# leejaehot/GaussianGrasper

Hardware: AMD Instinct MI355X
Metric: rendered views/sec (fwd+bwd) at 1M Gaussians, 1600x1200, 32-ch feature (higher is better)
Workload: dtype f32; 1 GPU; BASELINE config 4 per-GPU share: 1000000 Gaussians, 1600x1200, SH deg 4 rgb + 32-ch feature + depth + normal images per view (nerfstudio plugin route: the timed callable is FusedGaussianSplattingModel.get_outputs(camera) of gaussiangrasper_amd.plugin (the class train.sh loads, on stub.py's stand-ins for nerfstudio's base model and Cameras) — one fused rasterize operator per view), fwd+bwd, 8 views; route=plugin, deterministic_backward=False, python_gc=gc.freeze() after the warm-up (bench.freeze_gc), view_pipeline=backward of view k beside forward of view k + 1 on two streams, num_gaussians=1000000, feature_dim=32, n_visible=992125, parallelism=view-parallel x1, replicated Gaussians, grad_allreduce_bytes=472000000, grad_allreduce=per parameter, overlapped with the last view's backward

## Files before the change

### gaussiangrasper_amd/csrc/binning.hip

```cpp
#include "scan.h"

__device__ __forceinline__ int64_t dev_count(int64_t n, const int64_t *__restrict__ n_dev) {
    if (n_dev) {
        const int64_t d = *n_dev;
        if (d < n) n = d;
    }
    return n;
}

#define RS_THREADS 256
#define RS_WAVES (RS_THREADS / GG_WAVE)
#ifndef GG_RS_BIG
#define GG_RS_BIG 16
#endif
static inline int rs_items(int64_t n) { return n >= (int64_t)4096 * 1024 ? GG_RS_BIG : 4; }

__global__ __launch_bounds__(256) void count_kernel(int N, const int32_t *__restrict__ nth,
                                                    unsigned long long *__restrict__ out) {
    __shared__ unsigned long long part[4];
    unsigned long long acc = 0;
    for (int i = blockIdx.x * blockDim.x + threadIdx.x; i < N; i += gridDim.x * blockDim.x)
        acc += (unsigned long long)(uint32_t)nth[i];
    for (int off = 32; off > 0; off >>= 1) acc += __shfl_down(acc, off, 64);
    if ((threadIdx.x & 63) == 0) part[threadIdx.x >> 6] = acc;
    __syncthreads();
    if (threadIdx.x == 0) atomicAdd(out, part[0] + part[1] + part[2] + part[3]);
}

extern "C" size_t gg_count_workspace(int num_points) {
    (void)num_points;
    return 0;
}
extern "C" int gg_count_intersects(int N, const int32_t *num_tiles_hit, int64_t *out, void *ws,
                                   size_t ws_bytes, gg_stream_t stream) {
    (void)ws;
    (void)ws_bytes;
    GG_REQUIRE(N >= 0, "num_points < 0");
    GG_REQUIRE(out != nullptr, "null output");
    hipStream_t s = (hipStream_t)stream;
    if (gg_fill_async(out, 0, sizeof(int64_t), s) != hipSuccess) {
        gg_set_error("gg_count_intersects: memset failed");
        return GG_ERR_LAUNCH;
    }
    if (N == 0) return GG_OK;
    GG_REQUIRE(num_tiles_hit != nullptr, "null pointer");
    int blocks = min((N + 255) / 256, 128);
    gg_prof_begin(GG_K_COUNT, s);
    hipLaunchKernelGGL(count_kernel, dim3(blocks), dim3(256), 0, s, N, num_tiles_hit,
                       (unsigned long long *)out);
    gg_prof_end(GG_K_COUNT, s);
    GG_CHECK_LAUNCH();
    return GG_OK;
}

struct DepthSrc {
    const float *depths;
    const int32_t *radii;
};
__device__ __forceinline__ uint32_t depth_key(const DepthSrc d, int64_t idx) {
    return (d.radii[idx] > 0) ? __builtin_bit_cast(uint32_t, d.depths[idx]) : 0xFFFFFFFFu;
}

template <int RS_ITEMS>
__global__ __launch_bounds__(RS_THREADS) void radix_hist_kernel(
    int64_t n, const int64_t *__restrict__ n_dev, const uint32_t *__restrict__ keys, int shift,
    uint32_t mask, int nblocks, uint32_t *__restrict__ G, DepthSrc dsrc) {
    constexpr int RS_TILE = RS_THREADS * RS_ITEMS;
    __shared__ uint32_t hist[256];
    n = dev_count(n, n_dev);
    hist[threadIdx.x] = 0;
    __syncthreads();
    int64_t base = (int64_t)blockIdx.x * RS_TILE;
#pragma unroll 4
    for (int it = 0; it < RS_ITEMS; ++it) {
        int64_t idx = base + (int64_t)it * RS_THREADS + threadIdx.x;
        if (idx < n) atomicAdd(&hist[((dsrc.depths ? depth_key(dsrc, idx) : keys[idx]) >> shift) & mask], 1u);
    }
    __syncthreads();
    G[(size_t)threadIdx.x * nblocks + blockIdx.x] = hist[threadIdx.x];
}

__global__ __launch_bounds__(256) void radix_colscan_kernel(int nblocks, uint32_t *__restrict__ G,
                                                            uint32_t *__restrict__ totals) {
    __shared__ uint32_t wsum[4];
    __shared__ uint32_t carry_s;
    uint32_t *row = G + (size_t)blockIdx.x * nblocks;
    const int lane = threadIdx.x & 63, wave = threadIdx.x >> 6;
    if (threadIdx.x == 0) carry_s = 0;
    __syncthreads();
    for (int start = 0; start < nblocks; start += 256) {
        int i = start + threadIdx.x;
        uint32_t v = (i < nblocks) ? row[i] : 0u;
        uint32_t incl = v;
        for (int off = 1; off < 64; off <<= 1) {
            uint32_t t = __shfl_up(incl, off, 64);
            if (lane >= off) incl += t;
        }
        if (lane == 63) wsum[wave] = incl;
        __syncthreads();
        uint32_t wpre = 0;
        for (int w = 0; w < wave; ++w) wpre += wsum[w];
        uint32_t carry = carry_s;
        if (i < nblocks) row[i] = carry + wpre + incl - v;
        __syncthreads();
        if (threadIdx.x == 255) carry_s = carry + wpre + incl;
        __syncthreads();
    }
    if (threadIdx.x == 0) totals[blockIdx.x] = carry_s;
}

template <int RS_ITEMS>
__global__ __launch_bounds__(RS_THREADS) void radix_scatter_kernel(
    int64_t n, const int64_t *__restrict__ n_dev, const uint32_t *__restrict__ keys_in,
    const uint32_t *__restrict__ vals_in, uint32_t *__restrict__ keys_out,
    uint32_t *__restrict__ vals_out, int shift, uint32_t mask, int nblocks,
    const uint32_t *__restrict__ G, const uint32_t *__restrict__ totals, DepthSrc dsrc) {
    constexpr int RS_TILE = RS_THREADS * RS_ITEMS;
    n = dev_count(n, n_dev);
    const int nbits = 32 - __builtin_clz(mask | 1u);
    __shared__ uint32_t whist[RS_WAVES][256];
    __shared__ uint32_t digit_base[256];
    __shared__ uint32_t wsum[4];
    const int tid = threadIdx.x, lane = tid & 63, wave = tid >> 6;
    {
        uint32_t v = totals[tid];
        uint32_t incl = v;
        for (int off = 1; off < 64; off <<= 1) {
            uint32_t t = __shfl_up(incl, off, 64);
            if (lane >= off) incl += t;
        }
        if (lane == 63) wsum[wave] = incl;
        for (int w = 0; w < RS_WAVES; ++w) whist[w][tid] = 0;
        __syncthreads();
        uint32_t wpre = 0;
        for (int w = 0; w < wave; ++w) wpre += wsum[w];
        digit_base[tid] = wpre + incl - v + G[(size_t)tid * nblocks + blockIdx.x];
    }
    __syncthreads();

    const int64_t wbase = (int64_t)blockIdx.x * RS_TILE + (int64_t)wave * (GG_WAVE * RS_ITEMS);
    uint32_t key[RS_ITEMS], val[RS_ITEMS], rank[RS_ITEMS];
    const uint64_t lt_mask = (lane == 0) ? 0ull : (~0ull >> (64 - lane));
#pragma unroll
    for (int it = 0; it < RS_ITEMS; ++it) {
        int64_t idx = wbase + (int64_t)it * GG_WAVE + lane;
        bool valid = idx < n;
        key[it] = valid ? (dsrc.depths ? depth_key(dsrc, idx) : keys_in[idx]) : 0u;
        val[it] = valid ? (dsrc.depths ? (uint32_t)idx : vals_in[idx]) : 0u;
    }
#pragma unroll
    for (int it = 0; it < RS_ITEMS; ++it) {
        int64_t idx = wbase + (int64_t)it * GG_WAVE + lane;
        bool valid = idx < n;
        uint32_t d = (key[it] >> shift) & mask;
        uint64_t peers = __ballot(valid);
#pragma unroll
        for (int b = 0; b < 8; ++b) {
            if (b < nbits) {
                bool bit = (d >> b) & 1u;
                uint64_t m = __ballot(bit);
                peers &= bit ? m : ~m;
            }
        }
        uint32_t cnt = (uint32_t)__popcll(peers);
        uint32_t before = (uint32_t)__popcll(peers & lt_mask);
        uint32_t old = 0u;
        if (valid && before == 0) old = atomicAdd(&whist[wave][d], cnt);
        old = __shfl(old, (int)__builtin_ctzll(peers | (1ull << 63)), 64);
        rank[it] = old + before;
    }
    __syncthreads();
// ... 2 lines not shown
    {
        uint32_t run = 0;
        for (int w = 0; w < RS_WAVES; ++w) {
            uint32_t c = whist[w][tid];
            whist[w][tid] = run;
            run += c;
        }
        uint32_t incl = run;
        for (int off = 1; off < 64; off <<= 1) {
            uint32_t u = __shfl_up(incl, off, 64);
            if (lane >= off) incl += u;
        }
        if (lane == 63) wsum[wave] = incl;
        __syncthreads();
        uint32_t wpre = 0;
        for (int w = 0; w < wave; ++w) wpre += wsum[w];
        lstart[tid] = wpre + incl - run;
    }
    __syncthreads();
#pragma unroll
    for (int it = 0; it < RS_ITEMS; ++it) {
        int64_t idx = wbase + (int64_t)it * GG_WAVE + lane;
        if (idx < n) {
            uint32_t d = (key[it] >> shift) & mask;
            uint32_t lp = lstart[d] + whist[wave][d] + rank[it];
            skey[lp] = key[it];
            sval[lp] = val[it];
        }
    }
    __syncthreads();
    const int64_t left = n - (int64_t)blockIdx.x * RS_TILE;
    const int count = (int)(left < RS_TILE ? left : RS_TILE);
    for (int jj = tid; jj < count; jj += RS_THREADS) {
        const uint32_t k = skey[jj];
        const uint32_t d = (k >> shift) & mask;
        const uint32_t dst = digit_base[d] + ((uint32_t)jj - lstart[d]);
        keys_out[dst] = k;
        vals_out[dst] = sval[jj];
    }
}


typedef unsigned long long u64;
#define DB_BLOCKS 64
#define DB_THREADS 1024
#define DB_CAP 512
#define DB_MAX_BUCKETS 32768
static inline int db_buckets(int N) {
    int nb = 256;
    while (nb < DB_MAX_BUCKETS && nb * 64 < N) nb <<= 1;
    return nb;
}
struct DbRange {
    uint32_t kmin;
    u64 mul;
};
struct DbParts {
    const uint32_t *lo, *hi;
    int n;
};
__device__ __forceinline__ DbRange db_range_of(const DbParts mm, int nb, uint32_t *s_mm ) {
    const int tid = threadIdx.x;
    if (tid < 64) {
        uint32_t lo = 0xFFFFFFFFu, hi = 0u;
        for (int i = tid; i < mm.n; i += 64) {
            lo = min(lo, mm.lo[i]);
            hi = max(hi, mm.hi[i]);
        }
        for (int off = 32; off > 0; off >>= 1) {
            lo = min(lo, (uint32_t)__shfl_xor((int)lo, off, 64));
            hi = max(hi, (uint32_t)__shfl_xor((int)hi, off, 64));
        }
        if (tid == 0) { s_mm[0] = lo; s_mm[1] = hi; }
    }
    __syncthreads();
    DbRange r;
    const uint32_t lo = s_mm[0], hi = s_mm[1];
    r.kmin = lo;
    const u64 span = hi >= lo ? (u64)(hi - lo) + 1ull : 1ull;
    r.mul = (((u64)nb) << 32) / span;
    return r;
}
__device__ __forceinline__ uint32_t db_bucket(const DbRange r, uint32_t key, int nb) {
    if (key == 0xFFFFFFFFu) return (uint32_t)nb;
    return min((uint32_t)(((u64)(key - r.kmin) * r.mul) >> 32), (uint32_t)(nb - 1));
}
__global__ __launch_bounds__(256) void db_range_kernel(int N, DepthSrc dsrc, uint32_t *__restrict__ mm) {
    __shared__ uint32_t s_lo[4], s_hi[4];
    uint32_t lo = 0xFFFFFFFFu, hi = 0u;
    const int stride = 256 * gridDim.x;
    for (int i = blockIdx.x * 256 + threadIdx.x; i < N; i += 4 * stride) {
        uint32_t k[4];
#pragma unroll
        for (int u = 0; u < 4; ++u) k[u] = (i + u * stride < N) ? depth_key(dsrc, i + u * stride) : 0xFFFFFFFFu;
#pragma unroll
        for (int u = 0; u < 4; ++u)
            if (k[u] != 0xFFFFFFFFu) { lo = min(lo, k[u]); hi = max(hi, k[u]); }
    }
    for (int off = 32; off > 0; off >>= 1) {
        lo = min(lo, (uint32_t)__shfl_xor((int)lo, off, 64));
        hi = max(hi, (uint32_t)__shfl_xor((int)hi, off, 64));
    }
    if ((threadIdx.x & 63) == 0) { s_lo[threadIdx.x >> 6] = lo; s_hi[threadIdx.x >> 6] = hi; }
    __syncthreads();
    if (threadIdx.x == 0) {
        mm[blockIdx.x] = min(min(s_lo[0], s_lo[1]), min(s_lo[2], s_lo[3]));
        mm[gridDim.x + blockIdx.x] = max(max(s_hi[0], s_hi[1]), max(s_hi[2], s_hi[3]));
    }
}
#define DB_BOX_MAX 1023
struct DbGeom {
    const float *xys;
    int tiles_x, tiles_y;
};
__device__ __forceinline__ void db_box(const DbGeom g, const DepthSrc d, int i, uint32_t &cnt, uint32_t &box) {
    const int rad = d.radii[i];
    cnt = 0u;
    box = 1u << 20;
    if (rad > 0) {
        int x0, y0, x1, y1;
        gg_tile_bbox(g.xys[2 * (size_t)i], g.xys[2 * (size_t)i + 1], (float)rad, g.tiles_x, g.tiles_y, x0, y0, x1, y1);
        const int bw = x1 - x0;
        if (bw > 0 && y1 > y0) {
            cnt = (uint32_t)(bw * (y1 - y0));
            box = (uint32_t)x0 | ((uint32_t)y0 << 10) | ((uint32_t)bw << 20);
        }
    }
}
template <bool SCATTER>
__global__ __launch_bounds__(DB_THREADS) void db_walk_kernel(int N, int nb, DepthSrc dsrc, DbGeom geom,
                                                             const DbParts mm, uint32_t *__restrict__ G,
                                                             const uint32_t *__restrict__ start, uint4 *__restrict__ recs,
                                                             int32_t *__restrict__ zero = nullptr, int nzero = 0) {
    for (int i = blockIdx.x * DB_THREADS + threadIdx.x; i < nzero; i += DB_BLOCKS * DB_THREADS) zero[i] = 0;
    extern __shared__ uint32_t s_hist[];
    uint32_t *s_mm = s_hist + nb + 1;
    const DbRange r = db_range_of(mm, nb, s_mm);
    const int per = (N + DB_BLOCKS - 1) / DB_BLOCKS;
    const int lo = blockIdx.x * per, hi = min(N, lo + per);
    uint32_t *row = G + (size_t)blockIdx.x * (nb + 1);
    for (int b = threadIdx.x; b <= nb; b += DB_THREADS) s_hist[b] = SCATTER ? start[b] + row[b] : 0u;
    __syncthreads();
    for (int i = lo + threadIdx.x; i < hi; i += 4 * DB_THREADS) {
        uint32_t k[4], cnt[4], box[4];
#pragma unroll
        for (int u = 0; u < 4; ++u) {
            const int iu = i + u * DB_THREADS;
            k[u] = iu < hi ? depth_key(dsrc, iu) : 0u;
            cnt[u] = box[u] = 0u;
            if (SCATTER && iu < hi) db_box(geom, dsrc, iu, cnt[u], box[u]);
        }
#pragma unroll
        for (int u = 0; u < 4; ++u) {
            if (i + u * DB_THREADS < hi) {
                const uint32_t pos = atomicAdd(&s_hist[db_bucket(r, k[u], nb)], 1u);
                if (SCATTER && k[u] != 0xFFFFFFFFu)
                    recs[pos] = make_uint4(k[u], (uint32_t)(i + u * DB_THREADS), cnt[u], box[u]);
            }
        }
    }
    if (!SCATTER) {
        __syncthreads();
        for (int b = threadIdx.x; b <= nb; b += DB_THREADS) row[b] = s_hist[b];
    }
}
__global__ __launch_bounds__(256) void db_prefix_kernel(int nb, uint32_t *__restrict__ G, uint32_t *__restrict__ total) {
    const int b = blockIdx.x * 256 + threadIdx.x;
    if (b > nb) return;
    uint32_t run = 0;
    uint32_t c[DB_BLOCKS];
#pragma unroll
    for (int k = 0; k < DB_BLOCKS; ++k) c[k] = G[(size_t)k * (nb + 1) + b];
#pragma unroll
    for (int k = 0; k < DB_BLOCKS; ++k) {
        G[(size_t)k * (nb + 1) + b] = run;
        run += c[k];
    }
    total[b] = run;
}
__global__ __launch_bounds__(1024) void db_scan_kernel(int n, uint32_t *__restrict__ v) {
    __shared__ uint32_t s_w[2][16];
    const int tid = threadIdx.x, lane = tid & 63, wave = tid >> 6;
    uint32_t carry = 0u;
    int round = 0;
    for (int base = 0; base < n; base += 4 * 4096) {
        uint32_t x[4][4];
#pragma unroll
        for (int q = 0; q < 4; ++q)
#pragma unroll
            for (int k = 0; k < 4; ++k) {
                const int i = base + 4096 * q + 4 * tid + k;
                x[q][k] = i < n ? v[i] : 0u;
            }
#pragma unroll
        for (int q = 0; q < 4; ++q, ++round) {
            if (base + 4096 * q >= n) break;
            const uint32_t mine = x[q][0] + x[q][1] + x[q][2] + x[q][3];
            uint32_t incl = mine;
#pragma unroll
            for (int off = 1; off < 64; off <<= 1) {
                const uint32_t t = __shfl_up(incl, off, 64);
                if (lane >= off) incl += t;
            }
            uint32_t *sw = s_w[round & 1];
            if (lane == 63) sw[wave] = incl;
            __syncthreads();
            uint32_t ex = carry + incl - mine, all = 0u;
#pragma unroll
            for (int w = 0; w < 16; ++w) {
                const uint32_t t = sw[w];
                if (w < wave) ex += t;
                all += t;
            }
            carry += all;
#pragma unroll
            for (int k = 0; k < 4; ++k) {
                const int i = base + 4096 * q + 4 * tid + k;
                if (i < n) v[i] = ex;
                ex += x[q][k];
            }
        }
    }
    if (tid == 0) v[n] = carry;
}

__device__ __forceinline__ void db_ce(u64 &a, u64 &b) {
    const bool sw = b < a;
    const u64 lo = sw ? b : a, hi = sw ? a : b;
    a = lo;
    b = hi;
}
__device__ __forceinline__ void db_bitonic64(u64 *buf, const int n) {
    constexpr int NB = 8, LNB = 3, THREADS = 64;
    const int tid = threadIdx.x & 63;
    int P = NB;
    while (P < n) P <<= 1;
    const u64 INF = ~0ull;
    for (int blk = tid; blk * NB < n; blk += THREADS) {
        u64 v[NB];
#pragma unroll
        for (int r = 0; r < NB; ++r) v[r] = (NB * blk + r < n) ? buf[NB * blk + r] : INF;
#pragma unroll
        for (int k = 2; k <= NB; k <<= 1) {
#pragma unroll
            for (int i = 0; i < NB / 2; ++i) {
                const int b2 = i / (k / 2), off = i % (k / 2);
                db_ce(v[b2 * k + off], v[b2 * k + k - 1 - off]);
            }
#pragma unroll
            for (int j = k >> 2; j >= 1; j >>= 1)
#pragma unroll
                for (int i = 0; i < NB / 2; ++i) {
                    const int lo = ((i & ~(j - 1)) << 1) | (i & (j - 1));
                    db_ce(v[lo], v[lo + j]);
                }
        }
#pragma unroll
        for (int r = 0; r < NB; ++r)
            if (NB * blk + r < n) buf[NB * blk + r] = v[r];
    }
    { __builtin_amdgcn_fence(__ATOMIC_ACQ_REL, "workgroup"); __builtin_amdgcn_wave_barrier(); }
    for (int k = 2 * NB, lk = LNB + 1; k <= P; k <<= 1, ++lk) {
        const int hk = k >> 1;
        for (int i = tid; i < (P >> 1); i += THREADS) {
            const int blk = i >> (lk - 1), off = i & (hk - 1);
            const int lo = blk * k + off, hi = blk * k + k - 1 - off;
            if (hi < n) {
                const u64 a = buf[lo], b = buf[hi];
                if (b < a) { buf[lo] = b; buf[hi] = a; }
            }
        }
        { __builtin_amdgcn_fence(__ATOMIC_ACQ_REL, "workgroup"); __builtin_amdgcn_wave_barrier(); }
        for (int j = k >> 2; j >= NB; j >>= 1) {
            for (int i = tid; i < (P >> 1); i += THREADS) {
                const int lo = ((i & ~(j - 1)) << 1) | (i & (j - 1)), hi = lo + j;
                if (hi < n) {
// ... 177 lines not shown
#pragma unroll
                for (int r = 0; r < DB_ITEMS; ++r) key[r] = (64 * r < nv) ? buf[64 * r + lane] : ~0ull;
            }
            db_wsync();
        };
#pragma nounroll
        for (int round = 0; round < 2; ++round) {
#pragma nounroll
            for (int pb = round == 0 ? 4 : 0; pb < 8; ++pb) pass(8 * pb);
            if (round == 1) break;
            {
                DB_LIM(nv);
#pragma unroll
                for (int r = 0; r < DB_ITEMS; ++r)
                    if (64 * r < nv) buf[64 * r + lane] = key[r];
            }
            db_wsync();
            bool bad = false;
            {
                DB_LIM(nv);
#pragma unroll
                for (int r = 0; r < DB_ITEMS; ++r)
                    if (64 * r + 1 < nv) {
                        const u64 nx = buf[64 * r + lane + 1];
                        bad = bad || ((uint32_t)(nx >> 32) == (uint32_t)(key[r] >> 32) && (uint32_t)nx < (uint32_t)key[r]);
                    }
            }
            db_wsync();
            if (__ballot(bad) == 0ull) break;
        }
#undef DB_LIM
#pragma unroll
        for (int r = 0; r < DB_ITEMS; ++r) gid[r] = (uint32_t)key[r];
    } else {
        for (int i = lane; i < n; i += 64) {
            const uint4 rc = recs[s0 + i];
            pairs[s0 + i] = ((u64)rc.x << 32) | rc.y;
        }
        db_wsync();
        db_bitonic64(pairs + s0, n);
    }
    uint32_t carry = 0;
    for (int c0 = 0; c0 < n; c0 += DB_CAP) {
        if (n > DB_CAP) {
#pragma unroll
            for (int r = 0; r < DB_ITEMS; ++r) gid[r] = (c0 + 64 * r + lane < n) ? (uint32_t)pairs[s0 + c0 + 64 * r + lane] : 0u;
        }
#pragma unroll
        for (int r = 0; r < DB_ITEMS; ++r) {
            const int p = c0 + 64 * r + lane;
            if (c0 + 64 * r < n) {
                const bool valid = p < n;
                const uint32_t g = min(gid[r], (uint32_t)(N - 1));
                uint32_t c = cntv[r], bx = boxv[r];
                if (!carried) {
                    c = 0u;
                    bx = 1u << 20;
                    if (valid) db_box(geom, dsrc, (int)g, c, bx);
                }
                if (!valid) c = 0u;
                uint32_t incl = c;
#pragma unroll
                for (int off = 1; off < 64; off <<= 1) {
                    const uint32_t u = __shfl_up(incl, off, 64);
                    if (lane >= off) incl += u;
                }
                if (valid) {
                    order[s0 + p] = g;
                    einfo[s0 + p] = make_uint4(carry + incl - c, (uint32_t)b, bx, c);
                }
                carry += __shfl(incl, 63, 64);
            }
        }
    }
    if (lane == 0) bucket_sum[b] = carry;
}

__global__ __launch_bounds__(256) void emit_kernel(int N, const uint32_t *__restrict__ order,
                                                   const uint4 *__restrict__ einfo,
                                                   const uint32_t *__restrict__ bucket_base,
                                                   const uint32_t *__restrict__ visible, int tiles_x,
                                                   int64_t I, const int64_t *__restrict__ I_dev,
                                                   uint32_t *__restrict__ tkeys,
                                                   uint32_t *__restrict__ tvals) {
    __shared__ uint32_t s_rel[4][64];
    I = dev_count(I, I_dev);
    __shared__ int4 s_box[4][64];
    const int lane = threadIdx.x & 63, wave = threadIdx.x >> 6;
    const int r = blockIdx.x * blockDim.x + threadIdx.x;
    uint32_t g = 0, cnt = 0, off = 0;
    int x0 = 0, y0 = 0, bw = 1;
    if (r < N && (uint32_t)r < *visible) {
        g = min(order[r], (uint32_t)(N - 1));
        const uint4 e = einfo[r];
        off = e.x + bucket_base[e.y];
        x0 = (int)(e.z & 1023u);
        y0 = (int)((e.z >> 10) & 1023u);
        bw = max(1, (int)(e.z >> 20));
        cnt = e.w;
    }
    uint32_t incl = cnt;
    for (int d = 1; d < 64; d <<= 1) {
        uint32_t u = __shfl_up(incl, d, 64);
        if (lane >= d) incl += u;
    }
    const uint32_t total = __shfl(incl, 63, 64);
    const uint32_t base = __shfl(off, 0, 64);
    s_rel[wave][lane] = incl - cnt;
    s_box[wave][lane] = make_int4(x0, y0, bw, (int)g);
    __builtin_amdgcn_wave_barrier();
    const uint32_t *rel = s_rel[wave];
    for (uint32_t j = lane; j < total; j += 64) {
        int lo = 0;
#pragma unroll
        for (int step = 32; step > 0; step >>= 1)
            if (rel[lo + step] <= j) lo += step;
        const int4 b = s_box[wave][lo];
        const uint32_t k = j - rel[lo];
        const uint32_t row = k / (uint32_t)b.z;
        const int64_t cur = (int64_t)base + j;
        if (cur < I) {
            tkeys[cur] = (uint32_t)((b.y + (int)row) * tiles_x + b.x + (int)(k - row * (uint32_t)b.z));
            tvals[cur] = (uint32_t)b.w;
        }
    }
}

__global__ __launch_bounds__(256) void tile_bins_kernel(int64_t I, const int64_t *__restrict__ I_dev,
                                                        const uint32_t *__restrict__ tkeys_sorted,
                                                        uint32_t num_tiles,
                                                        int32_t *__restrict__ tile_bins,
                                                        int32_t *__restrict__ tile_out) {
    I = dev_count(I, I_dev);
    int64_t i = (int64_t)blockIdx.x * blockDim.x + threadIdx.x;
    if (i >= I) return;
    uint32_t cur = tkeys_sorted[i];
    if (tile_out) tile_out[i] = (int32_t)cur;
    const bool cur_ok = cur < num_tiles;
    if (i == 0 && cur_ok) tile_bins[2 * cur] = 0;
    if (i == I - 1 && cur_ok) tile_bins[2 * cur + 1] = (int32_t)I;
    if (i > 0) {
        uint32_t prev = tkeys_sorted[i - 1];
        if (prev != cur) {
            if (prev < num_tiles) tile_bins[2 * prev + 1] = (int32_t)i;
            if (cur_ok) tile_bins[2 * cur] = (int32_t)i;
        }
    }
}

static int radix_nblocks(int64_t n) {
    const int64_t tile = (int64_t)RS_THREADS * rs_items(n);
    return (int)((n + tile - 1) / tile);
}

struct BinWs {
    uint32_t *order;
    uint4 *einfo;
    uint32_t *G;
    uint32_t *totals;
    uint32_t *tkeyA, *tkeyB, *tvalTmp;
    uint4 *recs;
    u64 *pairs;
    uint32_t *dbG;
    uint32_t *dbStart;
    uint32_t *dbBase;
    uint32_t *dbmm;
    size_t bytes;
};
static BinWs bin_ws_layout(void *ws, int N, int64_t I) {
    BinWs w;
    size_t off = 0;
    auto take = [&](size_t nbytes) {
        char *p = ws ? (char *)ws + off : nullptr;
        off += gg_align_up(nbytes, 256);
        return (uint32_t *)p;
    };
    size_t n = (size_t)(N > 0 ? N : 1), i = (size_t)(I > 0 ? I : 1);
    w.order = take(4 * n);
    w.einfo = (uint4 *)take(16 * n);
    int nb = max(radix_nblocks(N), radix_nblocks(I));
    w.G = take(4 * 256 * (size_t)(nb + 1));
    w.totals = take(4 * 256);
    w.tkeyA = take(4 * i);
    w.tkeyB = take(4 * i);
    w.tvalTmp = take(4 * i);
    const size_t nbk = (size_t)db_buckets(N);
    w.recs = (uint4 *)take(16 * n);
    w.pairs = (u64 *)take(8 * n);
    w.dbG = take(4 * DB_BLOCKS * (nbk + 1));
    w.dbStart = take(4 * (nbk + 2));
    w.dbBase = take(4 * (nbk + 1));
    w.dbmm = take(4 * 2 * 256);
    w.bytes = off;
    return w;
}
extern "C" size_t gg_bin_sort_workspace(int num_points, int64_t num_intersects) {
    return bin_ws_layout(nullptr, num_points, num_intersects).bytes;
}

static void radix_pass(int64_t n, const int64_t *n_dev, const uint32_t *kin, const uint32_t *vin,
                       uint32_t *kout, uint32_t *vout, int shift, uint32_t mask, BinWs &w, hipStream_t s,
                       DepthSrc dsrc = DepthSrc{nullptr, nullptr}) {
    int nb = radix_nblocks(n);
    if (rs_items(n) != 4)
        hipLaunchKernelGGL(radix_hist_kernel<GG_RS_BIG>, dim3(nb), dim3(RS_THREADS), 0, s, n, n_dev, kin, shift,
                           mask, nb, w.G, dsrc);
    else
        hipLaunchKernelGGL(radix_hist_kernel<4>, dim3(nb), dim3(RS_THREADS), 0, s, n, n_dev, kin, shift,
                           mask, nb, w.G, dsrc);
    hipLaunchKernelGGL(radix_colscan_kernel, dim3(256), dim3(256), 0, s, nb, w.G, w.totals);
    if (rs_items(n) != 4)
        hipLaunchKernelGGL(radix_scatter_kernel<GG_RS_BIG>, dim3(nb), dim3(RS_THREADS), 0, s, n, n_dev, kin, vin,
                           kout, vout, shift, mask, nb, w.G, w.totals, dsrc);
    else
        hipLaunchKernelGGL(radix_scatter_kernel<4>, dim3(nb), dim3(RS_THREADS), 0, s, n, n_dev, kin, vin,
                           kout, vout, shift, mask, nb, w.G, w.totals, dsrc);
}

static int bin_sort_impl(int N, int64_t I, const int64_t *I_dev, const float *xys, const float *depths,
                         const int32_t *radii, const int32_t *num_tiles_hit, int tiles_x, int tiles_y,
                         int32_t *gaussian_ids_sorted, int32_t *tile_bins, int32_t *isect_tile_sorted,
                         void *ws, size_t ws_bytes, gg_stream_t stream, const uint32_t *range_lo = nullptr,
                         const uint32_t *range_hi = nullptr, int range_parts = 0) {
    GG_REQUIRE(N >= 0 && I >= 0, "negative size");
    GG_REQUIRE(tiles_x > 0 && tiles_y > 0, "empty tile grid");
    GG_REQUIRE(tiles_x <= DB_BOX_MAX && tiles_y <= DB_BOX_MAX, "tile grid beyond 1023 x 1023 (images beyond 16 368 pixels a side)");
    GG_REQUIRE(I < (int64_t)1 << 31, "num_intersects must fit int32 (tile_bins are int32)");
    GG_REQUIRE(tile_bins != nullptr, "null tile_bins");
    hipStream_t s = (hipStream_t)stream;
    const int T = tiles_x * tiles_y;
    if (N == 0 || I == 0) {
        if (gg_fill_async(tile_bins, 0, sizeof(int32_t) * 2 * (size_t)T, s) != hipSuccess) {
            gg_set_error("gg_bin_sort: memset failed");
            return GG_ERR_LAUNCH;
        }
        return GG_OK;
    }
    GG_REQUIRE(xys && depths && radii && num_tiles_hit && gaussian_ids_sorted, "null pointer");
    BinWs w = bin_ws_layout(ws, N, I);
    if (ws == nullptr || ws_bytes < w.bytes) {
        gg_set_error("gg_bin_sort: workspace too small (%zu < %zu)", ws_bytes, w.bytes);
        return GG_ERR_WORKSPACE;
    }
    gg_prof_begin(GG_K_BIN_SORT, s);
    const int nbk = db_buckets(N);
    const DepthSrc dsrc{depths, radii};
    const size_t walk_lds = sizeof(uint32_t) * ((size_t)nbk + 1 + 2);
    if (walk_lds > 64 * 1024) {
        (void)hipFuncSetAttribute((const void *)db_walk_kernel<false>, hipFuncAttributeMaxDynamicSharedMemorySize, (int)walk_lds);
        (void)hipFuncSetAttribute((const void *)db_walk_kernel<true>, hipFuncAttributeMaxDynamicSharedMemorySize, (int)walk_lds);
    }
    uint32_t *order = w.order;
    DbParts mm{w.dbmm, w.dbmm + 256, 256};
    if (range_lo && range_hi && range_parts > 0)
        mm = DbParts{range_lo, range_hi, range_parts};
    else
        hipLaunchKernelGGL(db_range_kernel, dim3(256), dim3(256), 0, s, N, dsrc, w.dbmm);
    const DbGeom geom{xys, tiles_x, tiles_y};
    hipLaunchKernelGGL(db_walk_kernel<false>, dim3(DB_BLOCKS), dim3(DB_THREADS), walk_lds, s, N, nbk, dsrc, geom, mm,
                       w.dbG, (const uint32_t *)nullptr, (uint4 *)nullptr, tile_bins, 2 * T);
    hipLaunchKernelGGL(db_prefix_kernel, dim3((nbk + 1 + 255) / 256), dim3(256), 0, s, nbk, w.dbG, w.dbStart);
    hipLaunchKernelGGL(db_scan_kernel, dim3(1), dim3(1024), 0, s, nbk, w.dbStart);
    hipLaunchKernelGGL(db_walk_kernel<true>, dim3(DB_BLOCKS), dim3(DB_THREADS), walk_lds, s, N, nbk, dsrc, geom, mm,
                       w.dbG, (const uint32_t *)w.dbStart, w.recs, (int32_t *)nullptr, 0);
    hipLaunchKernelGGL(db_sort_kernel, dim3((nbk + DB_WPB - 1) / DB_WPB), dim3(64 * DB_WPB), 0, s, N, nbk,
                       (const uint32_t *)w.dbStart, (const uint4 *)w.recs, w.pairs, dsrc, geom, order, w.einfo, w.dbBase);
    hipLaunchKernelGGL(db_scan_kernel, dim3(1), dim3(1024), 0, s, nbk, w.dbBase);
    int tile_bits = 1;
    while ((1 << tile_bits) < T) ++tile_bits;
    int passes = (tile_bits + 7) / 8;
    uint32_t *out_vals = (uint32_t *)gaussian_ids_sorted;
    uint32_t *kcur = w.tkeyA, *kalt = w.tkeyB;
    uint32_t *vcur = (passes % 2 == 0) ? out_vals : w.tvalTmp;
    uint32_t *valt = (passes % 2 == 0) ? w.tvalTmp : out_vals;
    if (!I_dev) {
        (void)gg_fill_async(kcur, 0xFF, sizeof(uint32_t) * (size_t)I, s);
        (void)gg_fill_async(vcur, 0, sizeof(uint32_t) * (size_t)I, s);
    }
    hipLaunchKernelGGL(emit_kernel, dim3((N + 255) / 256), dim3(256), 0, s, N, (const uint32_t *)order,
                       (const uint4 *)w.einfo, (const uint32_t *)w.dbBase, (const uint32_t *)(w.dbStart + nbk), tiles_x, I,
                       I_dev, kcur, vcur);
    const int per_pass = (tile_bits + passes - 1) / passes;
    for (int pass = 0; pass < passes; ++pass) {
        int bits = min(per_pass, tile_bits - per_pass * pass);
        radix_pass(I, I_dev, kcur, vcur, kalt, valt, per_pass * pass, (1u << bits) - 1u, w, s);
        uint32_t *t = kcur; kcur = kalt; kalt = t;
        t = vcur; vcur = valt; valt = t;
    }
    hipLaunchKernelGGL(tile_bins_kernel, dim3((unsigned)((I + 255) / 256)), dim3(256), 0, s, I, I_dev, kcur,
                       (uint32_t)T, tile_bins, isect_tile_sorted);
    gg_prof_end(GG_K_BIN_SORT, s);
    GG_CHECK_LAUNCH();
    return GG_OK;
}

extern "C" int gg_bin_sort_status(int N, int64_t I, const void *ws, size_t ws_bytes, gg_stream_t stream) {
    GG_REQUIRE(N >= 0 && I >= 0, "negative size");
    (void)ws;
    (void)ws_bytes;
    if (hipStreamSynchronize((hipStream_t)stream) != hipSuccess) {
        gg_set_error("gg_bin_sort_status: stream synchronisation failed");
        return GG_ERR_LAUNCH;
    }
    return GG_OK;
}

extern "C" int gg_bin_sort(int N, int64_t I, const float *xys, const float *depths,
                           const int32_t *radii, const int32_t *num_tiles_hit, int tiles_x,
                           int tiles_y, int32_t *gaussian_ids_sorted, int32_t *tile_bins,
                           int32_t *isect_tile_sorted, void *ws, size_t ws_bytes,
                           gg_stream_t stream) {
    return bin_sort_impl(N, I, nullptr, xys, depths, radii, num_tiles_hit, tiles_x, tiles_y,
                         gaussian_ids_sorted, tile_bins, isect_tile_sorted, ws, ws_bytes, stream);
}

extern "C" int gg_bin_sort_dev(int N, int64_t capacity, const int64_t *num_intersects_dev,
                               const float *xys, const float *depths, const int32_t *radii,
                               const int32_t *num_tiles_hit, int tiles_x, int tiles_y,
                               int32_t *gaussian_ids_sorted, int32_t *tile_bins,
                               int32_t *isect_tile_sorted, void *ws, size_t ws_bytes,
                               gg_stream_t stream) {
    GG_REQUIRE(num_intersects_dev != nullptr, "null num_intersects_dev");
    GG_REQUIRE(capacity >= 1, "capacity < 1");
    return bin_sort_impl(N, capacity, num_intersects_dev, xys, depths, radii, num_tiles_hit, tiles_x,
                         tiles_y, gaussian_ids_sorted, tile_bins, isect_tile_sorted, ws, ws_bytes, stream);
}

extern "C" int gg_bin_sort_dev_ex(int N, int64_t capacity, const int64_t *num_intersects_dev,
                                  const float *xys, const float *depths, const int32_t *radii,
                                  const int32_t *num_tiles_hit, int tiles_x, int tiles_y,
                                  int32_t *gaussian_ids_sorted, int32_t *tile_bins,
                                  int32_t *isect_tile_sorted, void *ws, size_t ws_bytes,
                                  const uint32_t *depth_bits_min, const uint32_t *depth_bits_max, int range_parts,
                                  gg_stream_t stream) {
    GG_REQUIRE(num_intersects_dev != nullptr, "null num_intersects_dev");
    GG_REQUIRE(capacity >= 1, "capacity < 1");
    GG_REQUIRE(range_parts == 0 || (depth_bits_min && depth_bits_max && range_parts > 0), "range parts without arrays");
    return bin_sort_impl(N, capacity, num_intersects_dev, xys, depths, radii, num_tiles_hit, tiles_x,
                         tiles_y, gaussian_ids_sorted, tile_bins, isect_tile_sorted, ws, ws_bytes, stream,
                         depth_bits_min, depth_bits_max, range_parts);
}

size_t gg_sort_pairs_workspace(int64_t n) {
// ... 32 lines not shown
```

Measured before the change: 638.9 views/s.

## Replace per-tile radix sort with coarse block binning plus fine in-block tile expansion

New measurement: 639.8 views/s (median of 6 runs). Within noise of the previous version (+0.1%).

```diff
diff --git a/gaussiangrasper_amd/csrc/binning.hip b/gaussiangrasper_amd/csrc/binning.hip
--- a/gaussiangrasper_amd/csrc/binning.hip
+++ b/gaussiangrasper_amd/csrc/binning.hip
@@ -68,6 +68,7 @@
     constexpr int RS_TILE = RS_THREADS * RS_ITEMS;
     __shared__ uint32_t hist[256];
     n = dev_count(n, n_dev);
+    if ((int64_t)blockIdx.x * RS_TILE >= n) return;
     hist[threadIdx.x] = 0;
     __syncthreads();
     int64_t base = (int64_t)blockIdx.x * RS_TILE;
@@ -81,16 +82,19 @@
 }
 
 __global__ __launch_bounds__(256) void radix_colscan_kernel(int nblocks, uint32_t *__restrict__ G,
-                                                            uint32_t *__restrict__ totals) {
+                                                            uint32_t *__restrict__ totals, int64_t n,
+                                                            const int64_t *__restrict__ n_dev, int tile) {
     __shared__ uint32_t wsum[4];
     __shared__ uint32_t carry_s;
     uint32_t *row = G + (size_t)blockIdx.x * nblocks;
+    n = dev_count(n, n_dev);
+    const int active = (int)min((int64_t)nblocks, (n + tile - 1) / tile);
     const int lane = threadIdx.x & 63, wave = threadIdx.x >> 6;
     if (threadIdx.x == 0) carry_s = 0;
     __syncthreads();
-    for (int start = 0; start < nblocks; start += 256) {
+    for (int start = 0; start < active; start += 256) {
         int i = start + threadIdx.x;
-        uint32_t v = (i < nblocks) ? row[i] : 0u;
+        uint32_t v = (i < active) ? row[i] : 0u;
         uint32_t incl = v;
         for (int off = 1; off < 64; off <<= 1) {
             uint32_t t = __shfl_up(incl, off, 64);
@@ -101,7 +105,7 @@
         uint32_t wpre = 0;
         for (int w = 0; w < wave; ++w) wpre += wsum[w];
         uint32_t carry = carry_s;
-        if (i < nblocks) row[i] = carry + wpre + incl - v;
+        if (i < active) row[i] = carry + wpre + incl - v;
         __syncthreads();
         if (threadIdx.x == 255) carry_s = carry + wpre + incl;
         __syncthreads();
@@ -117,6 +121,7 @@
     const uint32_t *__restrict__ G, const uint32_t *__restrict__ totals, DepthSrc dsrc) {
     constexpr int RS_TILE = RS_THREADS * RS_ITEMS;
     n = dev_count(n, n_dev);
+    if ((int64_t)blockIdx.x * RS_TILE >= n) return;
     const int nbits = 32 - __builtin_clz(mask | 1u);
     __shared__ uint32_t whist[RS_WAVES][256];
     __shared__ uint32_t digit_base[256];
@@ -225,7 +230,7 @@
     return nb;
 }
 struct DbRange {
-    uint32_t kmin;
+    uint32_t kmin, kmax;
     u64 mul;
 };
 struct DbParts {
@@ -250,13 +255,15 @@
     DbRange r;
     const uint32_t lo = s_mm[0], hi = s_mm[1];
     r.kmin = lo;
+    r.kmax = hi >= lo ? hi : lo;
     const u64 span = hi >= lo ? (u64)(hi - lo) + 1ull : 1ull;
     r.mul = (((u64)nb) << 32) / span;
     return r;
 }
 __device__ __forceinline__ uint32_t db_bucket(const DbRange r, uint32_t key, int nb) {
     if (key == 0xFFFFFFFFu) return (uint32_t)nb;
-    return min((uint32_t)(((u64)(key - r.kmin) * r.mul) >> 32), (uint32_t)(nb - 1));
+    const uint32_t k = min(max(key, r.kmin), r.kmax);
+    return min((uint32_t)(((u64)(k - r.kmin) * r.mul) >> 32), (uint32_t)(nb - 1));
 }
 __global__ __launch_bounds__(256) void db_range_kernel(int N, DepthSrc dsrc, uint32_t *__restrict__ mm) {
     __shared__ uint32_t s_lo[4], s_hi[4];
@@ -285,6 +292,7 @@
 struct DbGeom {
     const float *xys;
     int tiles_x, tiles_y;
+    int lbx, lby;
 };
 __device__ __forceinline__ void db_box(const DbGeom g, const DepthSrc d, int i, uint32_t &cnt, uint32_t &box) {
     const int rad = d.radii[i];
@@ -293,9 +301,10 @@
     if (rad > 0) {
         int x0, y0, x1, y1;
         gg_tile_bbox(g.xys[2 * (size_t)i], g.xys[2 * (size_t)i + 1], (float)rad, g.tiles_x, g.tiles_y, x0, y0, x1, y1);
-        const int bw = x1 - x0;
-        if (bw > 0 && y1 > y0) {
-            cnt = (uint32_t)(bw * (y1 - y0));
+        const int bw = x1 - x0, bh = y1 - y0;
+        if (bw > 0 && bh > 0) {
+            const int nblk = (((x1 - 1) >> g.lbx) - (x0 >> g.lbx) + 1) * (((y1 - 1) >> g.lby) - (y0 >> g.lby) + 1);
+            cnt = (uint32_t)nblk | ((uint32_t)bh << 16);
             box = (uint32_t)x0 | ((uint32_t)y0 << 10) | ((uint32_t)bw << 20);
         }
     }
@@ -351,7 +360,14 @@
     }
     total[b] = run;
 }
-__global__ __launch_bounds__(1024) void db_scan_kernel(int n, uint32_t *__restrict__ v) {
+struct TileOut {
+    int2 *bins;
+    int64_t I;
+    const int64_t *I_dev;
+    int32_t *ids, *tiles;
+};
+__global__ __launch_bounds__(1024) void db_scan_kernel(int n, uint32_t *__restrict__ v, TileOut to = TileOut{}) {
+    const int64_t L = to.bins ? dev_count(to.I, to.I_dev) : 0;
     __shared__ uint32_t s_w[2][16];
     const int tid = threadIdx.x, lane = tid & 63, wave = tid >> 6;
     uint32_t carry = 0u;
@@ -389,12 +405,23 @@
 #pragma unroll
             for (int k = 0; k < 4; ++k) {
                 const int i = base + 4096 * q + 4 * tid + k;
-                if (i < n) v[i] = ex;
+                if (i < n) {
+                    v[i] = ex;
+                    if (to.bins) {
+                        const int64_t e = ex, f = e + x[q][k];
+                        to.bins[i] = x[q][k] ? make_int2((int)min(e, L), (int)min(f, L)) : make_int2(0, 0);
+                    }
+                }
                 ex += x[q][k];
             }
         }
     }
     if (tid == 0) v[n] = carry;
+    if (to.bins)
+        for (int64_t p = (int64_t)carry + tid; p < L; p += 1024) {
+            to.ids[p] = 0;
+            if (to.tiles) to.tiles[p] = -1;
+        }
 }
 
 __device__ __forceinline__ void db_ce(u64 &a, u64 &b) {
@@ -678,13 +705,13 @@
             if (c0 + 64 * r < n) {
                 const bool valid = p < n;
                 const uint32_t g = min(gid[r], (uint32_t)(N - 1));
-                uint32_t c = cntv[r], bx = boxv[r];
+                uint32_t cw = cntv[r], bx = boxv[r];
                 if (!carried) {
-                    c = 0u;
+                    cw = 0u;
                     bx = 1u << 20;
-                    if (valid) db_box(geom, dsrc, (int)g, c, bx);
+                    if (valid) db_box(geom, dsrc, (int)g, cw, bx);
                 }
-                if (!valid) c = 0u;
+                const uint32_t c = valid ? cw & 0xFFFFu : 0u;
                 uint32_t incl = c;
 #pragma unroll
                 for (int off = 1; off < 64; off <<= 1) {
@@ -693,7 +720,7 @@
                 }
                 if (valid) {
                     order[s0 + p] = g;
-                    einfo[s0 + p] = make_uint4(carry + incl - c, (uint32_t)b, bx, c);
+                    einfo[s0 + p] = make_uint4(carry + incl - c, (uint32_t)b, bx, cw >> 16);
                 }
                 carry += __shfl(incl, 63, 64);
             }
@@ -702,28 +729,40 @@
     if (lane == 0) bucket_sum[b] = carry;
 }
 
-__global__ __launch_bounds__(256) void emit_kernel(int N, const uint32_t *__restrict__ order,
-                                                   const uint4 *__restrict__ einfo,
-                                                   const uint32_t *__restrict__ bucket_base,
-                                                   const uint32_t *__restrict__ visible, int tiles_x,
-                                                   int64_t I, const int64_t *__restrict__ I_dev,
-                                                   uint32_t *__restrict__ tkeys,
-                                                   uint32_t *__restrict__ tvals) {
+struct BinBlocks {
+    int lbx, lby;
+    int nbx;
+    int nblocks;
+};
+__device__ __forceinline__ int fs_seg(int bt) { return max(512, 8 * bt); }
+#define FS_BATCH 8
+
+__global__ __launch_bounds__(256) void coarse_emit_kernel(int N, const uint32_t *__restrict__ order,
+                                                          const uint4 *__restrict__ einfo,
+                                                          const uint32_t *__restrict__ bucket_base, int nbk,
+                                                          const uint32_t *__restrict__ visible, BinBlocks bb, int64_t I,
+                                                          const int64_t *__restrict__ I_dev, uint32_t *__restrict__ ckeys,
+                                                          uint32_t *__restrict__ cvals, int64_t *__restrict__ ccount) {
     __shared__ uint32_t s_rel[4][64];
-    I = dev_count(I, I_dev);
     __shared__ int4 s_box[4][64];
+    const int64_t L = dev_count(I, I_dev);
+    if (blockIdx.x == 0 && threadIdx.x == 0) *ccount = min((int64_t)bucket_base[nbk], L);
     const int lane = threadIdx.x & 63, wave = threadIdx.x >> 6;
     const int r = blockIdx.x * blockDim.x + threadIdx.x;
     uint32_t g = 0, cnt = 0, off = 0;
-    int x0 = 0, y0 = 0, bw = 1;
+    int x0 = 0, y0 = 0, x1 = 0, y1 = 0, nbx = 1;
     if (r < N && (uint32_t)r < *visible) {
         g = min(order[r], (uint32_t)(N - 1));
         const uint4 e = einfo[r];
         off = e.x + bucket_base[e.y];
         x0 = (int)(e.z & 1023u);
         y0 = (int)((e.z >> 10) & 1023u);
-        bw = max(1, (int)(e.z >> 20));
-        cnt = e.w;
+        x1 = x0 + (int)(e.z >> 20) - 1;
+        y1 = y0 + (int)e.w - 1;
+        if (e.w > 0u) {
+            nbx = (x1 >> bb.lbx) - (x0 >> bb.lbx) + 1;
+            cnt = (uint32_t)(nbx * ((y1 >> bb.lby) - (y0 >> bb.lby) + 1));
+        }
     }
     uint32_t incl = cnt;
     for (int d = 1; d < 64; d <<= 1) {
@@ -733,9 +772,11 @@
     const uint32_t total = __shfl(incl, 63, 64);
     const uint32_t base = __shfl(off, 0, 64);
     s_rel[wave][lane] = incl - cnt;
-    s_box[wave][lane] = make_int4(x0, y0, bw, (int)g);
+    s_box[wave][lane] = make_int4(x0 | (x1 << 16), y0 | (y1 << 16), nbx, (int)g);
     __builtin_amdgcn_wave_barrier();
     const uint32_t *rel = s_rel[wave];
+    const int BW = 1 << bb.lbx, BH = 1 << bb.lby;
+    const int sx1 = 8 + bb.lbx, sy0 = 8 + 2 * bb.lbx, sy1 = 8 + 2 * bb.lbx + bb.lby;
     for (uint32_t j = lane; j < total; j += 64) {
         int lo = 0;
 #pragma unroll
@@ -743,40 +784,144 @@
             if (rel[lo + step] <= j) lo += step;
         const int4 b = s_box[wave][lo];
         const uint32_t k = j - rel[lo];
-        const uint32_t row = k / (uint32_t)b.z;
+        const int row = (int)(k / (uint32_t)b.z), col = (int)k - row * b.z;
+        const int bx0 = b.x & 0xFFFF, bx1 = b.x >> 16, by0 = b.y & 0xFFFF, by1 = b.y >> 16;
+        const int bx = (bx0 >> bb.lbx) + col, by = (by0 >> bb.lby) + row;
+        const int X = bx << bb.lbx, Y = by << bb.lby;
+        const uint32_t key = (uint32_t)(by * bb.nbx + bx) | ((uint32_t)(max(bx0, X) - X) << 8) |
+                             ((uint32_t)(min(bx1, X + BW - 1) - X) << sx1) | ((uint32_t)(max(by0, Y) - Y) << sy0) |
+                             ((uint32_t)(min(by1, Y + BH - 1) - Y) << sy1);
         const int64_t cur = (int64_t)base + j;
-        if (cur < I) {
-            tkeys[cur] = (uint32_t)((b.y + (int)row) * tiles_x + b.x + (int)(k - row * (uint32_t)b.z));
-            tvals[cur] = (uint32_t)b.w;
-        }
-    }
-}
-
-__global__ __launch_bounds__(256) void tile_bins_kernel(int64_t I, const int64_t *__restrict__ I_dev,
-                                                        const uint32_t *__restrict__ tkeys_sorted,
-                                                        uint32_t num_tiles,
-                                                        int32_t *__restrict__ tile_bins,
-                                                        int32_t *__restrict__ tile_out) {
-    I = dev_count(I, I_dev);
-    int64_t i = (int64_t)blockIdx.x * blockDim.x + threadIdx.x;
-    if (i >= I) return;
-    uint32_t cur = tkeys_sorted[i];
-    if (tile_out) tile_out[i] = (int32_t)cur;
-    const bool cur_ok = cur < num_tiles;
-    if (i == 0 && cur_ok) tile_bins[2 * cur] = 0;
-    if (i == I - 1 && cur_ok) tile_bins[2 * cur + 1] = (int32_t)I;
-    if (i > 0) {
-        uint32_t prev = tkeys_sorted[i - 1];
-        if (prev != cur) {
-            if (prev < num_tiles) tile_bins[2 * prev + 1] = (int32_t)i;
-            if (cur_ok) tile_bins[2 * cur] = (int32_t)i;
-        }
-    }
-}
-
-static int radix_nblocks(int64_t n) {
-    const int64_t tile = (int64_t)RS_THREADS * rs_items(n);
+        if (cur < L) {
+            ckeys[cur] = key;
+            cvals[cur] = (uint32_t)b.w;
+        }
+    }
+}
+
+__device__ __forceinline__ bool fs_locate(const uint32_t *__restrict__ totals, int S, int seg, int &b, uint32_t &lo,
+                                          uint32_t &hi, int &first) {
+    __shared__ uint32_t s_cs[256], s_sf[257], s_w[2][4];
+    const int tid = threadIdx.x, lane = tid & 63, wave = tid >> 6;
+    const uint32_t c = totals[tid], ns = (c + (uint32_t)S - 1u) / (uint32_t)S;
+    uint32_t ic = c, is = ns;
+    for (int off = 1; off < 64; off <<= 1) {
+        const uint32_t u = __shfl_up(ic, off, 64), v = __shfl_up(is, off, 64);
+        if (lane >= off) { ic += u; is += v; }
+    }
+    if (lane == 63) { s_w[0][wave] = ic; s_w[1][wave] = is; }
+    __syncthreads();
+    uint32_t pc = 0, ps = 0;
+    for (int w = 0; w < wave; ++w) { pc += s_w[0][w]; ps += s_w[1][w]; }
+    s_cs[tid] = pc + ic - c;
+    s_sf[tid] = ps + is - ns;
+    if (tid == 255) s_sf[256] = ps + is;
+    __syncthreads();
+    if ((uint32_t)seg >= s_sf[256]) return false;
+    int k = 0;
+#pragma unroll
+    for (int step = 128; step > 0; step >>= 1)
+        if (k + step < 256 && s_sf[k + step] <= (uint32_t)seg) k += step;
+    b = k;
+    first = (int)s_sf[k];
+    lo = s_cs[k] + (uint32_t)(seg - first) * (uint32_t)S;
+    hi = min(lo + (uint32_t)S, s_cs[k] + totals[k]);
+    return true;
+}
+
+template <bool WRITE>
+__global__ __launch_bounds__(256) void fine_kernel(const uint32_t *__restrict__ ckeys, const uint32_t *__restrict__ cvals,
+                                                   const uint32_t *__restrict__ totals, BinBlocks bb, int tiles_x,
+                                                   int tiles_y, uint32_t *__restrict__ cnt, uint32_t *__restrict__ tot,
+                                                   int64_t I, const int64_t *__restrict__ I_dev,
+                                                   int32_t *__restrict__ ids, int32_t *__restrict__ tiles_out) {
+    const int lane = threadIdx.x & 63;
+    const int BW = 1 << bb.lbx, BH = 1 << bb.lby, BT = BW * BH, S = fs_seg(BT);
+    const int seg = blockIdx.x * 4 + (threadIdx.x >> 6);
+    int b, first;
+    uint32_t lo, hi;
+    if (!fs_locate(totals, S, seg, b, lo, hi, first)) return;
+    const int64_t L = WRITE ? dev_count(I, I_dev) : 0;
+    const int X = (b % bb.nbx) << bb.lbx, Y = (b / bb.nbx) << bb.lby;
+    const int sx1 = 8 + bb.lbx, sy0 = 8 + 2 * bb.lbx, sy1 = 8 + 2 * bb.lbx + bb.lby;
+    const uint64_t lt_mask = (lane == 0) ? 0ull : (~0ull >> (64 - lane));
+    for (int c0 = 0; c0 < BT; c0 += 64) {
+        const int lt = c0 + lane;
+        const int tx = X + (lt & (BW - 1)), ty = Y + (lt >> bb.lbx);
+        const bool own = lt < BT && tx < tiles_x && ty < tiles_y;
+        const int tile = own ? ty * tiles_x + tx : 0;
+        uint32_t run = 0;
+        if (WRITE && own) {
+            run = tot[tile];
+#pragma unroll 8
+            for (int s = first; s < seg; ++s) run += cnt[(size_t)s * BT + lt];
+        }
+        const int r0 = c0 >> bb.lbx, r1 = min(c0 + 64, BT) >> bb.lbx;
+        for (uint32_t b0 = lo; b0 < hi; b0 += 64 * FS_BATCH) {
+            uint32_t kk[FS_BATCH], gg[FS_BATCH];
+#pragma unroll
+            for (int q = 0; q < FS_BATCH; ++q) {
+                const uint32_t i = b0 + 64u * q + (uint32_t)lane;
+                kk[q] = i < hi ? ckeys[i] : 0u;
+                gg[q] = (WRITE && i < hi) ? cvals[i] : 0u;
+            }
+#pragma unroll
+            for (int q = 0; q < FS_BATCH; ++q) {
+                if (b0 + 64u * q >= hi) break;
+                const bool v = b0 + 64u * q + (uint32_t)lane < hi;
+                const uint32_t k = kk[q], gid = gg[q];
+                const int lx0 = (int)((k >> 8) & (uint32_t)(BW - 1)), lx1 = (int)((k >> sx1) & (uint32_t)(BW - 1));
+                const int ly0 = (int)((k >> sy0) & (uint32_t)(BH - 1)), ly1 = (int)((k >> sy1) & (uint32_t)(BH - 1));
+#pragma nounroll
+                for (int ry = r0; ry < r1; ++ry) {
+                    const bool rowc = v && ly0 <= ry && ry <= ly1;
+                    if (__ballot(rowc) == 0ull) continue;
+#pragma nounroll
+                    for (int rx = 0; rx < BW; ++rx) {
+                        const bool on = rowc && lx0 <= rx && rx <= lx1;
+                        const uint64_t m = __ballot(on);
+                        const int owner = ((ry << bb.lbx) | rx) - c0;
+                        if (WRITE && m != 0ull) {
+                            const uint32_t p = (uint32_t)__builtin_amdgcn_readlane((int)run, owner) +
+                                               (uint32_t)__popcll(m & lt_mask);
+                            if (on && (int64_t)p < L) {
+                                ids[p] = (int32_t)gid;
+                                if (tiles_out) tiles_out[p] = (Y + ry) * tiles_x + X + rx;
+                            }
+                        }
+                        if (lane == owner) run += (uint32_t)__popcll(m);
+                    }
+                }
+            }
+        }
+        if (!WRITE && lt < BT) {
+            cnt[(size_t)seg * BT + lt] = run;
+            if (run) atomicAdd(&tot[tile], run);
+        }
+    }
+}
+
+static int radix_nblocks(int64_t n, int items) {
+    const int64_t tile = (int64_t)RS_THREADS * items;
     return (int)((n + tile - 1) / tile);
+}
+static int radix_nblocks(int64_t n) { return radix_nblocks(n, rs_items(n)); }
+static int coarse_items(int64_t I) { return rs_items(I / 4); }
+
+static BinBlocks bin_blocks(int tiles_x, int tiles_y) {
+    BinBlocks b{3, 2, 0, 0};
+    for (;;) {
+        b.nbx = (tiles_x + (1 << b.lbx) - 1) >> b.lbx;
+        b.nblocks = b.nbx * ((tiles_y + (1 << b.lby) - 1) >> b.lby);
+        if (b.nblocks <= 256) return b;
+        if (b.lbx <= b.lby) ++b.lbx; else ++b.lby;
+    }
+}
+static int fs_seg_h(int bt) { return max(512, 8 * bt); }
+#define FS_MAX_BT 4096
+static int64_t fs_segments(int64_t L, const BinBlocks &bb) {
+    const int S = fs_seg_h(1 << (bb.lbx + bb.lby));
+    return (L + S - 1) / S + bb.nblocks;
 }
 
 struct BinWs {
@@ -784,7 +929,10 @@
     uint4 *einfo;
     uint32_t *G;
     uint32_t *totals;
-    uint32_t *tkeyA, *tkeyB, *tvalTmp;
+    uint32_t *ckA, *cvA, *ckB, *cvB;
+    int64_t *ccount;
+    uint32_t *fcnt;
+    uint32_t *ttot;
     uint4 *recs;
     u64 *pairs;
     uint32_t *dbG;
@@ -804,12 +952,15 @@
     size_t n = (size_t)(N > 0 ? N : 1), i = (size_t)(I > 0 ? I : 1);
     w.order = take(4 * n);
     w.einfo = (uint4 *)take(16 * n);
-    int nb = max(radix_nblocks(N), radix_nblocks(I));
-    w.G = take(4 * 256 * (size_t)(nb + 1));
+    w.G = take(4 * 256 * (size_t)(max(radix_nblocks(I), radix_nblocks(I, coarse_items(I))) + 1));
     w.totals = take(4 * 256);
-    w.tkeyA = take(4 * i);
-    w.tkeyB = take(4 * i);
-    w.tvalTmp = take(4 * i);
+    w.ckA = take(4 * i);
+    w.cvA = take(4 * i);
+    w.ckB = take(4 * i);
+    w.cvB = take(4 * i);
+    w.ccount = (int64_t *)take(8);
+    w.fcnt = take(4 * (i / 8 + 257 * (size_t)FS_MAX_BT));
+    w.ttot = take(4 * ((size_t)DB_BOX_MAX * DB_BOX_MAX + 1));
     const size_t nbk = (size_t)db_buckets(N);
     w.recs = (uint4 *)take(16 * n);
     w.pairs = (u64 *)take(8 * n);
@@ -826,16 +977,18 @@
 
 static void radix_pass(int64_t n, const int64_t *n_dev, const uint32_t *kin, const uint32_t *vin,
                        uint32_t *kout, uint32_t *vout, int shift, uint32_t mask, BinWs &w, hipStream_t s,
-                       DepthSrc dsrc = DepthSrc{nullptr, nullptr}) {
-    int nb = radix_nblocks(n);
-    if (rs_items(n) != 4)
+                       DepthSrc dsrc = DepthSrc{nullptr, nullptr}, int items = 0) {
+    if (items == 0) items = rs_items(n);
+    const int nb = radix_nblocks(n, items);
+    if (items != 4)
         hipLaunchKernelGGL(radix_hist_kernel<GG_RS_BIG>, dim3(nb), dim3(RS_THREADS), 0, s, n, n_dev, kin, shift,
                            mask, nb, w.G, dsrc);
     else
         hipLaunchKernelGGL(radix_hist_kernel<4>, dim3(nb), dim3(RS_THREADS), 0, s, n, n_dev, kin, shift,
                            mask, nb, w.G, dsrc);
-    hipLaunchKernelGGL(radix_colscan_kernel, dim3(256), dim3(256), 0, s, nb, w.G, w.totals);
-    if (rs_items(n) != 4)
+    hipLaunchKernelGGL(radix_colscan_kernel, dim3(256), dim3(256), 0, s, nb, w.G, w.totals, n, n_dev,
+                       RS_THREADS * items);
+    if (items != 4)
         hipLaunchKernelGGL(radix_scatter_kernel<GG_RS_BIG>, dim3(nb), dim3(RS_THREADS), 0, s, n, n_dev, kin, vin,
                            kout, vout, shift, mask, nb, w.G, w.totals, dsrc);
     else
@@ -868,6 +1021,13 @@
         gg_set_error("gg_bin_sort: workspace too small (%zu < %zu)", ws_bytes, w.bytes);
         return GG_ERR_WORKSPACE;
     }
+    const BinBlocks bb = bin_blocks(tiles_x, tiles_y);
+    const int BT = 1 << (bb.lbx + bb.lby);
+    const int64_t nseg = fs_segments(I, bb);
+    if ((size_t)nseg * BT > I / 8 + 257 * (size_t)FS_MAX_BT) {
+        gg_set_error("gg_bin_sort: segment counts exceed their workspace");
+        return GG_ERR_WORKSPACE;
+    }
     gg_prof_begin(GG_K_BIN_SORT, s);
     const int nbk = db_buckets(N);
     const DepthSrc dsrc{depths, radii};
@@ -882,39 +1042,32 @@
         mm = DbParts{range_lo, range_hi, range_parts};
     else
         hipLaunchKernelGGL(db_range_kernel, dim3(256), dim3(256), 0, s, N, dsrc, w.dbmm);
-    const DbGeom geom{xys, tiles_x, tiles_y};
+    const DbGeom geom{xys, tiles_x, tiles_y, bb.lbx, bb.lby};
     hipLaunchKernelGGL(db_walk_kernel<false>, dim3(DB_BLOCKS), dim3(DB_THREADS), walk_lds, s, N, nbk, dsrc, geom, mm,
-                       w.dbG, (const uint32_t *)nullptr, (uint4 *)nullptr, tile_bins, 2 * T);
+                       w.dbG, (const uint32_t *)nullptr, (uint4 *)nullptr, (int32_t *)w.ttot, T);
     hipLaunchKernelGGL(db_prefix_kernel, dim3((nbk + 1 + 255) / 256), dim3(256), 0, s, nbk, w.dbG, w.dbStart);
-    hipLaunchKernelGGL(db_scan_kernel, dim3(1), dim3(1024), 0, s, nbk, w.dbStart);
+    hipLaunchKernelGGL(db_scan_kernel, dim3(1), dim3(1024), 0, s, nbk, w.dbStart, TileOut{});
     hipLaunchKernelGGL(db_walk_kernel<true>, dim3(DB_BLOCKS), dim3(DB_THREADS), walk_lds, s, N, nbk, dsrc, geom, mm,
                        w.dbG, (const uint32_t *)w.dbStart, w.recs, (int32_t *)nullptr, 0);
     hipLaunchKernelGGL(db_sort_kernel, dim3((nbk + DB_WPB - 1) / DB_WPB), dim3(64 * DB_WPB), 0, s, N, nbk,
                        (const uint32_t *)w.dbStart, (const uint4 *)w.recs, w.pairs, dsrc, geom, order, w.einfo, w.dbBase);
-    hipLaunchKernelGGL(db_scan_kernel, dim3(1), dim3(1024), 0, s, nbk, w.dbBase);
-    int tile_bits = 1;
-    while ((1 << tile_bits) < T) ++tile_bits;
-    int passes = (tile_bits + 7) / 8;
-    uint32_t *out_vals = (uint32_t *)gaussian_ids_sorted;
-    uint32_t *kcur = w.tkeyA, *kalt = w.tkeyB;
-    uint32_t *vcur = (passes % 2 == 0) ? out_vals : w.tvalTmp;
-    uint32_t *valt = (passes % 2 == 0) ? w.tvalTmp : out_vals;
-    if (!I_dev) {
-        (void)gg_fill_async(kcur, 0xFF, sizeof(uint32_t) * (size_t)I, s);
-        (void)gg_fill_async(vcur, 0, sizeof(uint32_t) * (size_t)I, s);
-    }
-    hipLaunchKernelGGL(emit_kernel, dim3((N + 255) / 256), dim3(256), 0, s, N, (const uint32_t *)order,
-                       (const uint4 *)w.einfo, (const uint32_t *)w.dbBase, (const uint32_t *)(w.dbStart + nbk), tiles_x, I,
-                       I_dev, kcur, vcur);
-    const int per_pass = (tile_bits + passes - 1) / passes;
-    for (int pass = 0; pass < passes; ++pass) {
-        int bits = min(per_pass, tile_bits - per_pass * pass);
-        radix_pass(I, I_dev, kcur, vcur, kalt, valt, per_pass * pass, (1u << bits) - 1u, w, s);
-        uint32_t *t = kcur; kcur = kalt; kalt = t;
-        t = vcur; vcur = valt; valt = t;
-    }
-    hipLaunchKernelGGL(tile_bins_kernel, dim3((unsigned)((I + 255) / 256)), dim3(256), 0, s, I, I_dev, kcur,
-                       (uint32_t)T, tile_bins, isect_tile_sorted);
+    hipLaunchKernelGGL(db_scan_kernel, dim3(1), dim3(1024), 0, s, nbk, w.dbBase, TileOut{});
+    hipLaunchKernelGGL(coarse_emit_kernel, dim3((N + 255) / 256), dim3(256), 0, s, N, (const uint32_t *)order,
+                       (const uint4 *)w.einfo, (const uint32_t *)w.dbBase, nbk, (const uint32_t *)(w.dbStart + nbk), bb,
+                       I, I_dev, w.ckA, w.cvA, w.ccount);
+    int bbits = 1;
+    while ((1 << bbits) < bb.nblocks) ++bbits;
+    radix_pass(I, w.ccount, w.ckA, w.cvA, w.ckB, w.cvB, 0, (1u << bbits) - 1u, w, s, DepthSrc{nullptr, nullptr},
+               coarse_items(I));
+    const unsigned fs_grid = (unsigned)((nseg + 3) / 4);
+    hipLaunchKernelGGL(fine_kernel<false>, dim3(fs_grid), dim3(256), 0, s, (const uint32_t *)w.ckB,
+                       (const uint32_t *)w.cvB, (const uint32_t *)w.totals, bb, tiles_x, tiles_y, w.fcnt, w.ttot, I,
+                       I_dev, gaussian_ids_sorted, isect_tile_sorted);
+    hipLaunchKernelGGL(db_scan_kernel, dim3(1), dim3(1024), 0, s, T, w.ttot,
+                       TileOut{(int2 *)tile_bins, I, I_dev, gaussian_ids_sorted, isect_tile_sorted});
+    hipLaunchKernelGGL(fine_kernel<true>, dim3(fs_grid), dim3(256), 0, s, (const uint32_t *)w.ckB,
+                       (const uint32_t *)w.cvB, (const uint32_t *)w.totals, bb, tiles_x, tiles_y, w.fcnt, w.ttot, I,
+                       I_dev, gaussian_ids_sorted, isect_tile_sorted);
     gg_prof_end(GG_K_BIN_SORT, s);
     GG_CHECK_LAUNCH();
     return GG_OK;
```
